# pengsongyou/openscene

Hardware: AMD Instinct MI355X
Metric: active voxels/sec MinkUNet18A fwd+bwd @2cm ScanNet; per-point query ms (higher is better)
Workload: dtype f32 (bf16x6 split-precision MFMA, fp32 accumulate); 1 GPU; ScanNet distillation step (configs[2]): MinkUNet18A, 768-d head, 1 synthetic S100k scene/GPU (100999 voxels on rank 0, 2 cm), training-mode BN; timed = coordinate+kernel maps, forward, cosine loss, backward, gradient all-reduce, Adam step; arch=MinkUNet18A, feature_dim=768, voxels_rank0=100999, parallelism=dp1

## Files before the change

include/openscene_amd.h:

```cpp
#ifndef OPENSCENE_AMD_H
#define OPENSCENE_AMD_H

#include <stddef.h>
#include <stdint.h>

#ifdef __cplusplus
extern "C" {
#endif

#define OSN_OK 0
#define OSN_E_ARG (-1)
#define OSN_E_HIP (-2)
#define OSN_E_WS (-3)
#define OSN_E_RANGE (-4)

typedef void* osn_stream_t;

int osn_version(void);
const char* osn_last_error(void);
int osn_device_ok(void);

int64_t osn_hash_capacity(int64_t n);
size_t osn_coords_unique_ws_bytes(int64_t n);

// ... 460 lines not shown
int osn_net_backward(const osn_net_desc* net, const osn_net_run* run, osn_stream_t stream);
osn_events_t* osn_events_create(int n);
void osn_events_destroy(osn_events_t* e);

#define OSN_MAPS_MAX_STREAMS 4
typedef struct osn_map_level {
    const int32_t* coords4; const uint64_t* keys; const int32_t* vals;
    int64_t cap, rows;
} osn_map_level;
typedef struct osn_map_job {
    int32_t lvl_in, lvl_out;
    int32_t ksize, scale;
    int32_t self_map;
    int32_t stream;
    int32_t bm_fwd, bm_bwd;
    int32_t* nbr_fwd; int32_t* nbr_bwd; int64_t* counts;
    int32_t* order_fwd; int32_t* sorted_fwd; uint32_t* gmask_fwd;
    int32_t* order_bwd; int32_t* sorted_bwd; uint32_t* gmask_bwd;
    void* tl_fwd; void* tl_bwd; void* pl_fwd;
} osn_map_job;
int osn_maps_build(const osn_map_level* levels, int n_levels, const osn_map_job* jobs, int n_jobs,
                   const osn_stream_t* streams, void* const* ws, const uint64_t* ws_bytes, int n_streams,
                   osn_events_t* events);

osn_prof_t* osn_prof_create(int capacity);
void osn_prof_destroy(osn_prof_t* p);
int osn_prof_filter(osn_prof_t* p, const int32_t* tags, int n_tags);
int osn_prof_read(osn_prof_t* p, int32_t* tags, float* ms, int capacity, int reset);

#ifdef __cplusplus
}
#endif
#endif
```

openscene_amd/_lib.py:

```python
import ctypes
import os
import threading

_HERE = os.path.dirname(os.path.abspath(__file__))
LIB_PATH = os.environ.get("OSN_LIB_PATH") or os.path.join(_HERE, "lib", "libopenscene_amd.so")

_c = ctypes
_vp, _i32, _i64, _sz, _f32 = _c.c_void_p, _c.c_int, _c.c_int64, _c.c_size_t, _c.c_float

PROTOTYPES = {
    "osn_version": (_i32, []),
    "osn_last_error": (_c.c_char_p, []),
    "osn_device_ok": (_i32, []),
    "osn_hash_capacity": (_i64, [_i64]),
    "osn_coords_unique_ws_bytes": (_sz, [_i64]),
    "osn_coords_unique": (_i32, [_vp, _i64, _i32, _vp, _vp, _i64, _vp, _vp, _vp, _c.POINTER(_i64), _vp, _sz, _vp]),
    "osn_coords_unique_async": (_i32, [_vp, _i64, _vp, _i32, _vp, _vp, _i64, _vp, _vp, _vp, _vp, _vp, _vp, _sz, _vp]),
    "osn_coords_pyramid_async": (_i32, [_vp, _i64, _vp, _i32, _vp, _vp, _i64, _vp, _vp, _vp, _vp, _vp, _sz, _vp]),
    "osn_kmap_build": (_i32, [_vp, _vp, _i64, _vp, _i64, _i32, _i32, _vp, _vp, _vp]),
    "osn_kmap_build_self": (_i32, [_vp, _vp, _i64, _vp, _i64, _i32, _i32, _vp, _vp, _vp]),
    "osn_kmap_transpose": (_i32, [_vp, _i64, _i32, _i64, _vp, _vp]),
    "osn_kmap_sort_ws_bytes": (_sz, [_i64]),
    "osn_kmap_sort": (_i32, [_vp, _i64, _i32, _vp, _vp, _vp, _vp, _vp, _sz, _vp]),
    "osn_kmap_count": (_i32, [_vp, _i64, _i32, _vp, _vp]),
# ... 47 lines not shown
    "osn_seg_loss_bwd": (_i32, [_vp, _vp, _vp, _i64, _i32, _i64, _vp, _vp, _sz, _vp]),
    "osn_seg_loss_check": (_i32, [_vp, _i64, _i64, _i32, _vp]),
    "osn_seg_vote": (_i32, [_vp, _vp, _i64, _i64, _i32, _vp, _vp]),
    "osn_spconv_fwd_ws_ws_bytes": (_sz, [_i64, _i32, _i32, _i32]),
    "osn_spconv_fwd_ws": (_i32, [_vp, _i64, _vp, _vp, _i64, _i32, _i32, _vp, _vp, _i64, _i32, _i32, _i32, _vp, _sz, _vp]),
    "osn_spconv_wgrad_tl_partial": (_i32, [_vp, _vp, _vp, _i32, _vp, _i64, _i64, _i32, _i32, _i32, _vp, _sz, _vp, _vp]),
    "osn_wgrad_tl_reduce_batch": (_i32, [_vp, _i32, _vp]),
    "osn_stem_conv_fwd": (_i32, [_vp, _vp, _vp, _vp, _i64, _i32, _i32, _i32, _vp]),
    "osn_bn_ws_bytes": (_sz, [_i64, _i32]),
    "osn_bn_stats": (_i32, [_vp, _i64, _i32, _vp, _vp, _vp, _vp, _f32, _vp, _sz, _vp]),
    "osn_bn_apply": (_i32, [_vp, _vp, _vp, _vp, _vp, _f32, _vp, _i32, _vp, _vp, _i64, _i64, _i32, _vp]),
    "osn_spconv_fwd_rg_ok": (_i32, [_i64, _i32, _i32, _i32]),
    "osn_spconv_fwd_rg": (_i32, [_vp, _i64, _vp, _vp, _vp, _vp, _i64, _i32, _i32, _i32, _vp]),
    "osn_bn_forward_train": (_i32, [_vp, _i64, _i32, _vp, _vp, _f32, _vp, _i32, _f32, _vp, _vp, _vp, _vp, _vp, _vp, _i64, _vp, _sz, _vp]),
    "osn_bn_backward": (_i32, [_vp, _vp, _vp, _vp, _i32, _vp, _vp, _vp, _vp, _f32, _i32, _i32, _vp, _vp, _vp, _vp, _i64, _i32,
                               _vp, _sz, _vp]),
    "osn_bn_apply_plan": (_i32, [_i64, _i32, _c.POINTER(_i32), _c.POINTER(_i32)]),
    "osn_bn_set_flat_kernels": (_i32, [_i32]),
    "osn_bn_set_separate_finalize": (_i32, [_i32]),
    "osn_net_plan_query": (_i32, [_vp, _vp, _i32, _vp]),
    "osn_net_forward": (_i32, [_vp, _vp, _vp]),
    "osn_net_backward": (_i32, [_vp, _vp, _vp]),
    "osn_maps_build": (_i32, [_vp, _i32, _vp, _i32, _vp, _vp, _vp, _i32, _vp]),
    "osn_events_create": (_vp, [_i32]),
    "osn_events_destroy": (None, [_vp]),
    "osn_prof_create": (_vp, [_i32]),
    "osn_prof_destroy": (None, [_vp]),
    "osn_prof_filter": (_i32, [_vp, _vp, _i32]),
    "osn_prof_read": (_i32, [_vp, _vp, _vp, _i32, _i32]),
    "osn_relu_fwd": (_i32, [_vp, _vp, _i64, _vp]),
    "osn_relu_bwd": (_i32, [_vp, _vp, _vp, _i64, _vp]),
    "osn_add": (_i32, [_vp, _vp, _vp, _i64, _vp]),
    "osn_cat2": (_i32, [_vp, _i32, _vp, _i32, _vp, _i64, _vp]),
    "osn_cat2_bwd": (_i32, [_vp, _vp, _i32, _vp, _i32, _i64, _vp]),
    "osn_cosine_query": (_i32, [_vp, _vp, _vp, _vp, _vp, _i64, _i32, _i32, _vp]),
    "osn_query_ensemble_ws_bytes": (_sz, [_i64]),
    "osn_query_ensemble": (_i32, [_vp, _vp, _vp, _vp, _vp, _vp, _vp, _vp, _i64, _i32, _i32, _vp, _sz, _vp]),
    "osn_cosine_query_vote": (_i32, [_vp, _vp, _vp, _vp, _vp, _i64, _i32, _i32, _vp]),
    "osn_query_ensemble_vote": (_i32, [_vp, _vp, _vp, _vp, _vp, _vp, _vp, _vp, _i64, _i32, _i32, _vp, _sz, _vp]),
    "osn_eval_confusion": (_i32, [_vp, _vp, _i64, _i32, _vp, _vp, _i64, _vp, _i32, _vp, _vp, _i32, _vp]),
    "osn_eval_check": (_i32, [_vp, _vp]),
    "osn_bank_append": (_i32, [_vp, _i64, _vp, _i64, _i32, _vp, _i64, _vp, _vp]),
    "osn_bank_check": (_i32, [_vp, _vp]),
    "osn_bank_search_ws_bytes": (_sz, [_i64, _i32, _i32, _i32, _i64]),
    "osn_bank_search": (_i32, [_vp, _i64, _i32, _vp, _i32, _i64, _vp, _i32, _i32, _i32, _vp, _vp, _vp, _vp, _vp, _vp, _vp, _sz, _vp]),
    "osn_bank_append_fp8": (_i32, [_vp, _i32, _i64, _vp, _i64, _i32, _vp, _vp, _i64, _vp, _vp]),
# ... 113 lines not shown
```

openscene_amd/csrc/coords.hip:

```cpp
#include "common.h"
#include "coords_impl.h"

namespace osn {

constexpr int SCAN_TPB = 256;
constexpr int SCAN_IPT = 4;
constexpr int SCAN_BLOCK = SCAN_TPB * SCAN_IPT;

__device__ inline int wave_incl_scan(int v, int lane) {
#pragma unroll
    for (int d = 1; d < 64; d <<= 1) {
        int t = __shfl_up(v, d, 64);
        if (lane >= d) v += t;
    }
    return v;
}

template <bool FLAG>
__global__ __launch_bounds__(SCAN_TPB) void scan_block_kernel(const int* __restrict__ in, int* __restrict__ out,
                                                              int* __restrict__ sums, int64_t n,
                                                              const int32_t* __restrict__ n_dev, const int32_t* __restrict__ vals,
                                                              const int32_t* __restrict__ slot_of, int* __restrict__ flag_out) {
    if (n_dev) n = *n_dev;
    __shared__ int wave_tot[SCAN_TPB / 64];
// ... 193 lines not shown
        return;
    }
    int r = -1;
    if (o < n) {
        const int ix = k % ksize, iy = (k / ksize) % ksize, iz = k / (ksize * ksize);
        const int c = ksize / 2;
        const int4 p = coords[o];
        const int x = p.y + (ix - c) * scale, y = p.z + (iy - c) * scale, z = p.w + (iz - c) * scale;
        const int lim = COORD_BIAS - 1;
        if (x >= -lim && x <= lim && y >= -lim && y <= lim && z >= -lim && z <= lim)
            r = table_find(keys, vals, mask, pack_key(p.x, x, y, z));
        nbr[int64_t(k) * n + o] = r;
        if (r >= 0) nbr[int64_t(K - 1 - k) * n + r] = int(o);
    }
    if (counts) {
        const int c = __syncthreads_count(r >= 0);
        if (threadIdx.x == 0 && c) {
            atomicAdd(&counts[k], (unsigned long long)c);
            atomicAdd(&counts[K - 1 - k], (unsigned long long)c);
        }
    }
}

__global__ void kmap_transpose_kernel(const int32_t* __restrict__ nbr, int64_t n_out, int64_t n_in,
                                      int32_t* __restrict__ tbl) {
    const int64_t o = int64_t(blockIdx.x) * blockDim.x + threadIdx.x;
    const int k = blockIdx.y;
    if (o >= n_out) return;
    const int i = nbr[int64_t(k) * n_out + o];
    if (i >= 0) tbl[int64_t(k) * n_in + i] = int(o);
}

__global__ void kmap_count_kernel(const int32_t* __restrict__ nbr, int64_t n_out, unsigned long long* counts) {
    const int k = blockIdx.y;
    int64_t c = 0;
    for (int64_t o = int64_t(blockIdx.x) * blockDim.x + threadIdx.x; o < n_out; o += int64_t(gridDim.x) * blockDim.x)
        c += nbr[int64_t(k) * n_out + o] >= 0;
    __shared__ long long wsum[4];
    for (int d = 32; d >= 1; d >>= 1) c += __shfl_down(c, d, 64);
    if ((threadIdx.x & 63) == 0) wsum[threadIdx.x >> 6] = c;
    __syncthreads();
    if (threadIdx.x == 0) {
        const long long t = wsum[0] + wsum[1] + wsum[2] + wsum[3];
        if (t) atomicAdd(&counts[k], (unsigned long long)t);
    }
}
// ... 219 lines not shown
                                   int64_t* counts, osn_stream_t stream) {
    return kmap_build_self_impl(table_keys, table_vals, cap, coords4, n, ksize, offset_scale, nbr, counts, false, static_cast<hipStream_t>(stream));
}

int osn::kmap_build_self_impl(const uint64_t* table_keys, const int32_t* table_vals, int64_t cap, const int32_t* coords4, int64_t n,
                              int ksize, int offset_scale, int32_t* nbr, int64_t* counts, bool prefilled, hipStream_t st) {
    OSN_REQUIRE(ksize >= 1 && ksize <= 7 && (ksize & 1) == 1, OSN_E_ARG, "osn_kmap_build_self: ksize=%d must be odd, <= 7", ksize);
    OSN_REQUIRE(cap >= 2 && (cap & (cap - 1)) == 0, OSN_E_ARG, "osn_kmap_build_self: cap must be a power of two");
    OSN_REQUIRE(n >= 0, OSN_E_ARG, "osn_kmap_build_self: n < 0");
    const int K = ksize * ksize * ksize;
    if (counts && !prefilled) OSN_HIP(hipMemsetAsync(counts, 0, size_t(K) * 8, st));
    if (n == 0) return OSN_OK;
    OSN_REQUIRE(table_keys && table_vals && coords4 && nbr, OSN_E_ARG, "osn_kmap_build_self: null pointer");
    OSN_REQUIRE(aligned16(coords4), OSN_E_ARG, "osn_kmap_build_self: coords4 must be 16-byte aligned");
    if (K > 1 && !prefilled) OSN_HIP(hipMemsetAsync(nbr + int64_t(K / 2 + 1) * n, 0xFF, size_t(K / 2) * size_t(n) * 4, st));
    const int T = 256;
    hipLaunchKernelGGL(kmap_build_self_kernel, dim3(cdiv(n, T), K / 2 + 1), dim3(T), 0, st, table_keys, table_vals,
                       uint32_t(cap - 1), reinterpret_cast<const int4*>(coords4), n, ksize, offset_scale, nbr,
                       reinterpret_cast<unsigned long long*>(counts));
    OSN_LAUNCH_CHECK();
    return OSN_OK;
}

extern "C" int osn_kmap_transpose(const int32_t* nbr, int64_t n_out, int K, int64_t n_in, int32_t* tbl,
                                  osn_stream_t stream) {
    return kmap_transpose_impl(nbr, n_out, K, n_in, tbl, false, static_cast<hipStream_t>(stream));
}

int osn::kmap_transpose_impl(const int32_t* nbr, int64_t n_out, int K, int64_t n_in, int32_t* tbl, bool prefilled, hipStream_t st) {
    OSN_REQUIRE(K >= 1 && n_out >= 0 && n_in >= 0, OSN_E_ARG, "osn_kmap_transpose: bad sizes");
    if (n_in == 0) return OSN_OK;
    OSN_REQUIRE(tbl, OSN_E_ARG, "osn_kmap_transpose: null tbl");
    if (!prefilled) OSN_HIP(hipMemsetAsync(tbl, 0xFF, size_t(K) * size_t(n_in) * 4, st));
    if (n_out == 0) return OSN_OK;
    OSN_REQUIRE(nbr, OSN_E_ARG, "osn_kmap_transpose: null nbr");
    const int T = 256;
    hipLaunchKernelGGL(kmap_transpose_kernel, dim3(cdiv(n_out, T), K), dim3(T), 0, st, nbr, n_out, n_in, tbl);
    OSN_LAUNCH_CHECK();
    return OSN_OK;
}

extern "C" int osn_kmap_count(const int32_t* nbr, int64_t n_out, int K, int64_t* counts, osn_stream_t stream) {
    hipStream_t st = static_cast<hipStream_t>(stream);
    OSN_REQUIRE(K >= 1 && n_out >= 0 && counts, OSN_E_ARG, "osn_kmap_count: bad arguments");
    OSN_HIP(hipMemsetAsync(counts, 0, size_t(K) * 8, st));
    if (n_out == 0) return OSN_OK;
// ... 10 lines not shown
```

openscene_amd/csrc/coords_impl.h:

```cpp
#pragma once
#include "common.h"

namespace osn {

struct FillJob {
    void* ptr;
    uint64_t bytes;
    uint32_t value;
    uint32_t pad;
};
constexpr int FILL_BATCH = 48;
struct FillJobs {
    FillJob j[FILL_BATCH];
};
int fill_batch(const FillJob* jobs, int n, hipStream_t st);

int kmap_build_impl(const uint64_t* in_table_keys, const int32_t* in_table_vals, int64_t cap, const int32_t* out_coords4, int64_t n_out,
                    int ksize, int offset_scale, int32_t* nbr, int64_t* counts, bool prefilled, hipStream_t st);
int kmap_build_self_impl(const uint64_t* table_keys, const int32_t* table_vals, int64_t cap, const int32_t* coords4, int64_t n, int ksize,
                         int offset_scale, int32_t* nbr, int64_t* counts, bool prefilled, hipStream_t st);
int kmap_transpose_impl(const int32_t* nbr, int64_t n_out, int K, int64_t n_in, int32_t* tbl, bool prefilled, hipStream_t st);

}
```

openscene_amd/csrc/maps.hip:

```cpp
#include "common.h"
#include "events.h"
#include "coords_impl.h"
#include <vector>

using namespace osn;

extern "C" int osn_maps_build(const osn_map_level* levels, int n_levels, const osn_map_job* jobs, int n_jobs,
                              const osn_stream_t* streams, void* const* ws, const uint64_t* ws_bytes, int n_streams,
                              osn_events_t* events) {
    OSN_REQUIRE(levels && jobs && streams && ws && ws_bytes && n_levels >= 1 && n_jobs >= 0 && n_streams >= 1 &&
                    n_streams <= OSN_MAPS_MAX_STREAMS,
                OSN_E_ARG, "osn_maps_build: bad arguments (%d levels, %d jobs, %d streams)", n_levels, n_jobs, n_streams);
    OSN_REQUIRE(n_streams == 1 || (events && events_count(events) >= n_streams + 1), OSN_E_ARG,
                "osn_maps_build: %d streams need an event pool of at least %d events", n_streams, n_streams + 1);
    hipStream_t main = static_cast<hipStream_t>(streams[0]);
    {
        std::vector<FillJob> fills;
        for (int j = 0; j < n_jobs; ++j) {
            const osn_map_job& q = jobs[j];
            if (q.lvl_in < 0 || q.lvl_in >= n_levels || q.lvl_out < 0 || q.lvl_out >= n_levels || q.ksize < 1 || q.ksize > 7 || !q.nbr_fwd) continue;
            const int K = q.ksize * q.ksize * q.ksize;
            const int64_t n_in = levels[q.lvl_in].rows;
            if (q.counts) fills.push_back(FillJob{q.counts, uint64_t(K) * 8u, 0u, 0u});
            if (q.self_map) {
                if (K > 1 && n_in > 0) fills.push_back(FillJob{q.nbr_fwd + int64_t(K / 2 + 1) * n_in, uint64_t(K / 2) * uint64_t(n_in) * 4u, 0xFFFFFFFFu, 0u});
            } else if (q.nbr_bwd && n_in > 0) {
                fills.push_back(FillJob{q.nbr_bwd, uint64_t(K) * uint64_t(n_in) * 4u, 0xFFFFFFFFu, 0u});
            }
        }
        const int rc = fill_batch(fills.data(), int(fills.size()), main);
        if (rc) return rc;
    }
    if (n_streams > 1) {
        hipEvent_t e0 = events_get(events, 0);
        OSN_HIP(hipEventRecord(e0, main));
        for (int s = 1; s < n_streams; ++s) OSN_HIP(hipStreamWaitEvent(static_cast<hipStream_t>(streams[s]), e0, 0));
    }
    bool used[OSN_MAPS_MAX_STREAMS] = {false};
    for (int j = 0; j < n_jobs; ++j) {
        const osn_map_job& q = jobs[j];
        OSN_REQUIRE(q.lvl_in >= 0 && q.lvl_in < n_levels && q.lvl_out >= 0 && q.lvl_out < n_levels && q.ksize >= 1 && q.ksize <= 7,
                    OSN_E_ARG, "osn_maps_build: job %d: levels / kernel size", j);
        const int si = q.stream >= 0 && q.stream < n_streams ? q.stream : 0;
        used[si] = true;
        osn_stream_t st = streams[si];
        const osn_map_level& li = levels[q.lvl_in];
        const osn_map_level& lo = levels[q.lvl_out];
        const int K = q.ksize * q.ksize * q.ksize;
        OSN_REQUIRE(q.nbr_fwd && li.rows >= 1 && lo.rows >= 1, OSN_E_ARG, "osn_maps_build: job %d: null table or empty level", j);
        int rc;
        if (q.self_map) {
            OSN_REQUIRE(q.lvl_in == q.lvl_out && (q.ksize & 1), OSN_E_ARG, "osn_maps_build: job %d: a self map needs one level and an odd kernel", j);
            rc = kmap_build_self_impl(li.keys, li.vals, li.cap, li.coords4, li.rows, q.ksize, q.scale, q.nbr_fwd, q.counts, true,
                                      static_cast<hipStream_t>(st));
        } else {
            rc = kmap_build_impl(li.keys, li.vals, li.cap, lo.coords4, lo.rows, q.ksize, q.scale, q.nbr_fwd, q.counts, true,
                                 static_cast<hipStream_t>(st));
            if (!rc && q.nbr_bwd) rc = kmap_transpose_impl(q.nbr_fwd, lo.rows, K, li.rows, q.nbr_bwd, true, static_cast<hipStream_t>(st));
        }
        if (rc) return rc;
        if (q.sorted_fwd) {
            rc = osn_kmap_sort(q.nbr_fwd, lo.rows, K, q.counts, q.order_fwd, q.sorted_fwd, q.gmask_fwd, ws[si], size_t(ws_bytes[si]), st);
            if (rc) return rc;
        }
        if (q.sorted_bwd) {
            OSN_REQUIRE(q.nbr_bwd, OSN_E_ARG, "osn_maps_build: job %d: tile order of a missing input-gradient table", j);
            rc = osn_kmap_sort(q.nbr_bwd, li.rows, K, q.counts, q.order_bwd, q.sorted_bwd, q.gmask_bwd, ws[si], size_t(ws_bytes[si]), st);
            if (rc) return rc;
        }
        if (q.tl_fwd) {
            rc = osn_tile_lists_build(q.sorted_fwd ? q.sorted_fwd : q.nbr_fwd, lo.rows, K, q.bm_fwd, q.tl_fwd, st);
            if (rc) return rc;
            if (q.pl_fwd) {
                rc = osn_pair_lists_build(q.tl_fwd, q.sorted_fwd ? q.order_fwd : nullptr, lo.rows, K, q.bm_fwd, q.pl_fwd, st);
                if (rc) return rc;
            }
        }
// ... 15 lines not shown
```

openscene_amd/csrc/wgrad_tl.hip:

```cpp
#include "common.h"
#include "split.h"
#include <cstdlib>
#include "pairlist.h"

namespace osn {

typedef short s16x4 __attribute__((ext_vector_type(4)));

__device__ inline int wave_incl_scan_i32(int v, int lane) {
#pragma unroll
    for (int d = 1; d < 64; d <<= 1) {
        const int t = __shfl_up(v, d, 64);
        if (lane >= d) v += t;
    }
    return v;
}

__global__ __launch_bounds__(256) void pair_prefix_kernel(const int32_t* __restrict__ cnt, int n_tiles, int K,
                                                          int32_t* __restrict__ pref, int32_t* __restrict__ total) {
    __shared__ int wtot[4];
    __shared__ int carry_s;
    const int k = blockIdx.x, tid = threadIdx.x, lane = tid & 63, wave = tid >> 6;
    if (tid == 0) carry_s = 0;
    __syncthreads();
    for (int t0 = 0; t0 < n_tiles; t0 += 256) {
        const int t = t0 + tid;
        const int v = t < n_tiles ? cnt[int64_t(t) * K + k] : 0;
        const int incl = wave_incl_scan_i32(v, lane);
        if (lane == 63) wtot[wave] = incl;
        __syncthreads();
        int woff = 0;
#pragma unroll
        for (int w = 0; w < 4; ++w) woff += w < wave ? wtot[w] : 0;
        const int carry = carry_s;
        if (t < n_tiles) pref[int64_t(k) * n_tiles + t] = carry + woff + incl - v;
        __syncthreads();
        if (tid == 255) carry_s = carry + woff + incl;
        __syncthreads();
    }
    if (tid == 0) total[k] = carry_s;
}

__global__ __launch_bounds__(256) void pair_fill_kernel(const int32_t* __restrict__ cnt, const int2* __restrict__ lst,
                                                        const int32_t* __restrict__ out_rows,
                                                        const int32_t* __restrict__ pref, const int32_t* __restrict__ total,
                                                        int n_tiles, int K, int bm, int32_t* __restrict__ pin,
                                                        int32_t* __restrict__ pout, int32_t* __restrict__ poff) {
    __shared__ int poff_s[PL_KMAX + 1];
    const int tid = threadIdx.x, lane = tid & 63, wave = tid >> 6;
    const int64_t tile = blockIdx.x;
    if (wave == 0) {
        int carry = 0;
        for (int k0 = 0; k0 < K; k0 += 64) {
            const int k = k0 + lane;
            const int v = k < K ? total[k] : 0;
            const int incl = wave_incl_scan_i32(v, lane);
            if (k < K) poff_s[k] = carry + incl - v;
            carry += __shfl(incl, 63, 64);
        }
        if (lane == 0) poff_s[K] = carry;
    }
    __syncthreads();
    if (tile == 0)
        for (int k = tid; k <= K; k += 256) poff[k] = poff_s[k];
    for (int k = wave; k < K; k += 4) {
        const int c = cnt[tile * K + k];
        const int base = poff_s[k] + pref[int64_t(k) * n_tiles + tile];
        const int2* src = lst + (tile * K + k) * bm;
        for (int p = lane; p < c; p += 64) {
            const int2 e = src[p];
            pin[base + p] = e.x;
            const int64_t r = tile * bm + e.y;
            pout[base + p] = out_rows ? out_rows[r] : int(r);
        }
    }
}

__global__ __launch_bounds__(256) void pair_plan_kernel(const int32_t* __restrict__ total, int K, int4* __restrict__ items,
                                                        int2* __restrict__ range, int items_max) {
    __shared__ int nk[PL_KMAX];
    __shared__ int start[PL_KMAX + 1];
    __shared__ int quota_s;
    const int tid = threadIdx.x;
    if (tid == 0) {
        long long P = 0;
        for (int k = 0; k < K; ++k) P += total[k];
        long long q = (P + (items_max - K) - 1) / (items_max - K);
        q = (q + 31) / 32 * 32;
        if (q < PL_MIN_QUOTA) q = PL_MIN_QUOTA;
        quota_s = int(q);
    }
    __syncthreads();
    const int quota = quota_s;
    if (tid < K) nk[tid] = (total[tid] + quota - 1) / quota;
    __syncthreads();
    if (tid == 0) {
        int acc = 0;
        for (int k = 0; k < K; ++k) { start[k] = acc; acc += nk[k]; }
        start[K] = acc;
    }
    __syncthreads();
    if (tid < K) range[tid] = make_int2(start[tid], start[tid + 1]);
    for (int t = tid; t < PL_ITEMS; t += 256) {
        int4 it = make_int4(-1, 0, 0, 0);
        if (t < start[K]) {
            int k = 0;
            while (k + 1 < K && start[k + 1] <= t) ++k;
            const int j = t - start[k];
            it.x = k;
            it.y = j * quota;
            it.z = min(it.y + quota, total[k]);
        }
        items[t] = it;
    }
}

template <int MB, int NB, bool BUFG = false>
__global__ __launch_bounds__(256, 2) void wgrad_tl_kernel(const float* __restrict__ rows_a, const float* __restrict__ rows_g,
                                                          const int32_t* __restrict__ idx_a, const int32_t* __restrict__ idx_g,
                                                          const int32_t* __restrict__ poff, const int4* __restrict__ items,
                                                          float* __restrict__ partial, int ca, int cg, int n_cgb,
                                                          int ident_rows, int ident_quota, unsigned a_bytes, unsigned g_bytes) {
    constexpr int CA_T = 32 * MB, CG_T = 32 * NB;
    constexpr int LDA = CA_T + 8, LDG = CG_T + 8;
    constexpr int QA = CA_T / 4, QG = CG_T / 4;
    __shared__ __attribute__((aligned(16))) __bf16 Ap[3][32][LDA];
    __shared__ __attribute__((aligned(16))) __bf16 Gp[3][32][LDG];
    __shared__ int idxbuf[2][32];

    const int tid = threadIdx.x, lane = tid & 63;
    const int wave = __builtin_amdgcn_readfirstlane(tid >> 6);
    const int wi = wave >> 1, wj = wave & 1;
    const int a0 = (blockIdx.x / n_cgb) * CA_T;
    const int g0 = (blockIdx.x % n_cgb) * CG_T;
    int k, p0, p1, base;
    int pstep = 32;
    if (idx_a) {
// ... 218 lines not shown
    return pl_view(nullptr, n_out, K, bm).bytes;
}

extern "C" int osn_pair_lists_build(const void* tl, const int32_t* out_rows, int64_t n_out, int K, int bm, void* pl,
                                    osn_stream_t stream) {
    hipStream_t st = static_cast<hipStream_t>(stream);
    OSN_REQUIRE(n_out >= 0 && n_out < (int64_t(1) << 31), OSN_E_ARG, "osn_pair_lists_build: n_out out of range");
    OSN_REQUIRE(K >= 1 && K <= PL_KMAX && bm >= 1, OSN_E_ARG, "osn_pair_lists_build: K=%d bm=%d", K, bm);
    OSN_REQUIRE(int64_t(K) * n_out < (int64_t(1) << 31), OSN_E_ARG, "osn_pair_lists_build: K * n_out exceeds 32-bit pair indices");
    OSN_REQUIRE(pl, OSN_E_ARG, "osn_pair_lists_build: null pointer");
    PlView v = pl_view(pl, n_out, K, bm);
    if (n_out == 0) {
        OSN_HIP(hipMemsetAsync(pl, 0, PL_OFF_ITEMS, st));
        OSN_HIP(hipMemsetAsync(v.items, 0xFF, size_t(PL_ITEMS) * 16, st));
        OSN_HIP(hipMemsetAsync(v.range, 0, size_t(PL_KMAX) * 8, st));
        return OSN_OK;
    }
    OSN_REQUIRE(tl, OSN_E_ARG, "osn_pair_lists_build: null tile lists");
    const int64_t nt = cdiv(n_out, bm);
    const int32_t* cnt = static_cast<const int32_t*>(tl);
    const int2* lst = reinterpret_cast<const int2*>(static_cast<const char*>(tl) + align_up(size_t(nt) * K * 4, 256));
    hipLaunchKernelGGL(pair_prefix_kernel, dim3(K), dim3(256), 0, st, cnt, int(nt), K, v.pref, v.total);
    const int items_max = PL_ITEMS;
    hipLaunchKernelGGL(pair_plan_kernel, dim3(1), dim3(256), 0, st, v.total, K, v.items, v.range, items_max);
    hipLaunchKernelGGL(pair_fill_kernel, dim3(unsigned(nt)), dim3(256), 0, st, cnt, lst, out_rows, v.pref, v.total, int(nt), K,
                       bm, v.pin, v.pout, v.poff);
    OSN_LAUNCH_CHECK();
    return OSN_OK;
}

namespace {
struct WgTlPlan {
    int mb, nb, n_ab, n_gb;
};
WgTlPlan plan_wg_tl(int ca, int cg) {
    auto blocks = [](int c) { int t = (c + 31) / 32; return t > 4 ? 4 : t; };
    WgTlPlan p;
    p.mb = blocks(ca);
    p.nb = blocks(cg);
    p.n_ab = int(cdiv(ca, 32 * p.mb));
    p.n_gb = int(cdiv(cg, 32 * p.nb));
    return p;
}
int ident_quota(int64_t n) {
    int64_t q = cdiv(n, PL_ITEMS);
    q = (q + 31) / 32 * 32;
    if (q < 64) q = 64;
    return int(q);
}
// ... 142 lines not shown
```

openscene_amd/ops.py:

```python
import ctypes
import os
import threading
import weakref

import torch

from . import _lib
from ._lib import check

_vp = ctypes.c_void_p

_profiler = None


def set_profiler(p):
    global _profiler
    _profiler = p


_raw_stream_of = torch._C._cuda_getCurrentRawStream
_current_device = torch._C._cuda_getDevice


def _prof_start(kind, dev, **meta):
# ... 252 lines not shown

_MAP_LEVEL = None
_MAP_JOB = None
_map_events = {}
MAPS_STREAMS = int(os.environ.get("OSN_MAPS_STREAMS", "1"))


def _map_dtypes():
    global _MAP_LEVEL, _MAP_JOB
    if _MAP_LEVEL is None:
        import numpy as np
        _MAP_LEVEL = np.dtype([("coords4", "<u8"), ("keys", "<u8"), ("vals", "<u8"), ("cap", "<i8"), ("rows", "<i8")])
        _MAP_JOB = np.dtype([(n, "<i4") for n in ("lvl_in", "lvl_out", "ksize", "scale", "self_map", "stream", "bm_fwd", "bm_bwd")] +
                            [(n, "<u8") for n in ("nbr_fwd", "nbr_bwd", "counts", "order_fwd", "sorted_fwd", "gmask_fwd", "order_bwd",
                                                  "sorted_bwd", "gmask_bwd", "tl_fwd", "tl_bwd", "pl_fwd")])
        assert _MAP_LEVEL.itemsize == 40 and _MAP_JOB.itemsize == 128
    return _MAP_LEVEL, _MAP_JOB


def _addr(v):
    return 0 if v is None else (int(v) if isinstance(v, int) else v.data_ptr())


def maps_build(levels, jobs, dev, sort_rows, streams=None):
    import numpy as np
    lib = _prep(dev)
    ldt, jdt = _map_dtypes()
    la = np.zeros(len(levels), dtype=ldt)
    for i, (c, t, rows) in enumerate(levels):
        la[i] = (c.data_ptr(), t.keys.data_ptr(), t.vals.data_ptr(), t.cap, rows)
    ja = np.zeros(max(len(jobs), 1), dtype=jdt)
    for i, q in enumerate(jobs):
        ja[i] = tuple((_addr(q.get(n)) if jdt[n].kind == "u" else int(q.get(n, 0))) for n in jdt.names)
    ns = max(1, min(int(streams) if streams else MAPS_STREAMS, 3))
    idx = _idx(dev)
    main = _stream(dev)
    raws = [main]
    if ns > 1:
        pool = [s for s in (side_stream(dev), aux_stream(dev)) if s.cuda_stream != main]
        ns = min(ns, 1 + len(pool))
        raws += [s.cuda_stream for s in pool[:ns - 1]]
        ev = _map_events.get(idx)
        if ev is None:
            with _Dev(dev):
                ev = _map_events[idx] = lib.osn_events_create(8)
        if not ev:
            ns, raws, ev = 1, [main], None
    else:
        ev = None
    wsb = int(_cached("osn_kmap_sort_ws_bytes", int(sort_rows))) if sort_rows else 256
    wss = [_ws(wsb, dev)] + [ws_on(wsb, dev, r) for r in raws[1:]]
    st_arr = (ctypes.c_void_p * ns)(*raws)
    ws_arr = (ctypes.c_void_p * ns)(*[w.data_ptr() for w in wss])
    wb_arr = (ctypes.c_uint64 * ns)(*[w.numel() for w in wss])
    with _Dev(dev):
        check(lib.osn_maps_build(la.ctypes.data, len(levels), ja.ctypes.data, len(jobs), st_arr, ws_arr, wb_arr, ns, ev),
              "osn_maps_build")


def _w3(weight):
    return weight.unsqueeze(0) if weight.dim() == 2 else weight


def _table_conv(kind, lib, feats, wptr, nbr, n_out, out_rows, gmask, K, cin, cout):
    dev = feats.device
    if nbr is not None:
        if nbr.dtype != torch.int32 or nbr.shape != (K, n_out):
            raise ValueError("nbr must be int32 [%d, %d], got %s %s" % (K, n_out, nbr.dtype, tuple(nbr.shape)))
        nbr = nbr.contiguous()
    elif K != 1 or feats.shape[0] != n_out:
        raise ValueError("nbr=None is the identity map and needs K == 1 and n_in == n_out")
    out = torch.empty((n_out, cout), dtype=torch.float32, device=dev)
    wsb = _cached("osn_spconv_fwd_ws_bytes", n_out, K, cin, cout)
    ws = _ws(wsb, dev) if wsb else None
    tok = _prof_start(kind, dev, n_in=feats.shape[0], n_out=n_out, K=K, cin=cin, cout=cout)
    with _Dev(dev):
        check(getattr(lib, "osn_" + kind)(_p(feats), wptr, _p(nbr), _p(out_rows), _p(gmask), _p(out), n_out, K, cin, cout,
                                          _p(ws), int(wsb), _stream(dev)), "osn_" + kind)
    if tok is not None:
        _profiler.stop(tok)
# ... 2157 lines not shown
```

openscene_amd/sparse.py:

```python
import torch

from . import ops


def _F_mod():
    from . import functional
    return functional


class CoordinateManager:

    PYRAMID = (2, 4, 8, 16)

    def __init__(self, coordinates, pyramid=None):
        pyramid = self.PYRAMID if pyramid is None else tuple(pyramid)
        levels = ops.coords_pyramid(coordinates, (1,) + pyramid)
        coords, inverse, first, table = levels[0]
        self.n_input = coordinates.shape[0]
        self.unique_index = None
        self.inverse_mapping = None
        if coords.shape[0] != coordinates.shape[0]:
            self.unique_index = first.long()
            self.inverse_mapping = inverse.long()
        else:
# ... 107 lines not shown
                continue
            K, n_in, n_out = k ** 3, self.size(si), self.size(so)
            own = si == so
            e = dict(key=key, K=K, n_in=n_in, n_out=n_out, own=own, lane=lane.get((si, so, k), 0), lvl_in=index[si], lvl_out=index[so],
                     ksize=k, scale=si)
            e["nbr_fwd"] = take(4 * K * n_out)
            e["counts"] = take(8 * K)
            if not own:
                e["nbr_bwd"] = take(4 * K * n_in)
            for side, rows, on in (("fwd", n_out, True), ("bwd", n_in, not own)):
                if on and self._want_sort(K, rows):
                    e["order_" + side], e["sorted_" + side] = take(4 * rows), take(4 * K * rows)
                    e["gmask_" + side] = take(4 * ((rows + 31) // 32))
                    sort_rows = max(sort_rows, rows)
                if on and K <= 32:
                    bm = ops.tile_rows(rows)
                    e["bm_" + side] = bm
                    e["tl_" + side] = take(ops._cached("osn_tile_lists_bytes", rows, K, bm))
            if "tl_fwd" in e and (pairs is True or (pairs == "ws" and ((k == 2 and so == 2 * si) or n_out <= _F_mod().WS_MAX_ROWS))):
                e["pl_fwd"] = take(ops._cached("osn_pair_lists_bytes", n_out, K, e["bm_fwd"]))
            plan.append(e)
        if not plan:
            return
        arena = torch.empty(total, dtype=torch.uint8, device=dev)
        base = arena.data_ptr()
        ptr_fields = ("nbr_fwd", "nbr_bwd", "counts", "order_fwd", "sorted_fwd", "gmask_fwd", "order_bwd", "sorted_bwd", "gmask_bwd",
                      "tl_fwd", "tl_bwd", "pl_fwd")
        jobs = []
        for e in plan:
            q = dict(lvl_in=e["lvl_in"], lvl_out=e["lvl_out"], ksize=e["ksize"], scale=e["scale"], self_map=int(e["own"]), stream=e["lane"],
                     bm_fwd=e.get("bm_fwd", 0), bm_bwd=e.get("bm_bwd", 0))
            for f in ptr_fields:
                if f in e:
                    q[f] = base + e[f][0]
            jobs.append(q)
        ops.maps_build([(self._coords[s], self._tables[s], self.size(s)) for s in levels], jobs, dev, sort_rows, streams)

        def view(e, f, dtype, shape):
            off, nb = e[f]
            return arena[off:off + nb].view(dtype).view(shape)
        for e in plan:
            K, n_in, n_out, key = e["K"], e["n_in"], e["n_out"], e["key"]
            nbr = view(e, "nbr_fwd", torch.int32, (K, n_out))
            counts = view(e, "counts", torch.int64, (K,))
            bwd = nbr if e["own"] else view(e, "nbr_bwd", torch.int32, (K, n_in))
            tiles = {}
            for side, rows in (("fwd", n_out), ("bwd", n_in)):
                tiles[side] = (view(e, "order_" + side, torch.int32, (rows,)), view(e, "sorted_" + side, torch.int32, (K, rows)),
                               view(e, "gmask_" + side, torch.int32, ((rows + 31) // 32,))) if ("order_" + side) in e else None
            if e["own"]:
                tiles["bwd"] = tiles["fwd"]
            self._kmaps[key] = (nbr, bwd, bool(e["own"]))
            self._kmaps[("counts",) + key] = counts
            self._kmaps[("tiles",) + key] = (tiles["fwd"], tiles["bwd"])
            if "tl_fwd" in e:
                lf = ops.TileLists(view(e, "tl_fwd", torch.uint8, (e["tl_fwd"][1],)), e["bm_fwd"], n_out, K,
                                   tiles["fwd"][0] if tiles["fwd"] is not None else None)
                lb = lf if e["own"] else ops.TileLists(view(e, "tl_bwd", torch.uint8, (e["tl_bwd"][1],)), e["bm_bwd"], n_in, K,
                                                       tiles["bwd"][0] if tiles["bwd"] is not None else None)
# ... 5 lines not shown
        seen = []

        def walk(v):
            if isinstance(v, torch.Tensor):
                seen.append(v)
            elif isinstance(v, (tuple, list)):
                for u in v:
                    walk(u)
            elif isinstance(v, ops.HashTable):
                walk((v.keys, v.vals))
            elif isinstance(v, ops.TileLists):
                walk((v.buf, v.out_rows))
        for d in (self._coords, self._tables, self._parent, self._kmaps):
            for v in d.values():
                walk(v)
        return seen

    def record_stream(self, stream):
        for t in self.tensors():
            t.record_stream(stream)

    SORT_MIN_ROWS = 8192
    SORT_MIN_ROWS_K8 = 10 ** 9

    def kmap_tiles(self, in_stride, out_stride, ksize, dilation=1):
        key = ("tiles", in_stride, out_stride, ksize, dilation)
        hit = self._kmaps.get(key)
        if hit is not None:
            return hit
        fwd, bwd, flip = self.kmap(in_stride, out_stride, ksize, dilation)
        counts = self.kmap_counts(in_stride, out_stride, ksize, dilation)

        def tiles(tbl):
            if tbl is None or tbl.shape[0] > 32 or tbl.shape[1] < self.SORT_MIN_ROWS:
                return None
            if tbl.shape[0] <= 8 and tbl.shape[1] < self.SORT_MIN_ROWS_K8:
                return None
            return ops.kmap_sort(tbl, counts)

        tf = tiles(fwd)
        tb = tf if (bwd is fwd) else tiles(bwd)
        res = (tf, tb)
        self._kmaps[key] = res
        return res


# ... 155 lines not shown
```

Measured before the change: 12.98 million voxels/s.

## Build self kernel maps via 4x4x4 occupancy bitmap and derive 3x3 from 5x5

Adds an occupancy hash of 64-bit bricks, each bit marking one voxel of a 4x4x4 block. Self kernel-map builds test this bitmap first and probe the main hash table only for offsets that are occupied, which avoids most empty-neighbour lookups. A 3x3x3 self map is copied out of an existing 5x5x5 map on the same level instead of being rebuilt. The pair-plan kernel is also folded into pair_fill, saving one launch. The cost is extra arena memory, a memset of the occupancy table and a fill pass, plus more complex code paths that can be switched off with a legacy flag.

```diff
diff --git a/include/openscene_amd.h b/include/openscene_amd.h
--- a/include/openscene_amd.h
+++ b/include/openscene_amd.h
@@ -506,6 +506,11 @@
 int osn_maps_build(const osn_map_level* levels, int n_levels, const osn_map_job* jobs, int n_jobs,
                    const osn_stream_t* streams, void* const* ws, const uint64_t* ws_bytes, int n_streams,
                    osn_events_t* events);
+size_t osn_maps_occupancy_bytes(int64_t rows);
+int osn_maps_build_occ(const osn_map_level* levels, int n_levels, const osn_map_job* jobs, int n_jobs,
+                       const osn_stream_t* streams, void* const* ws, const uint64_t* ws_bytes, int n_streams,
+                       osn_events_t* events, void* const* occ);
+int osn_maps_set_legacy(int on);
 
 osn_prof_t* osn_prof_create(int capacity);
 void osn_prof_destroy(osn_prof_t* p);
diff --git a/openscene_amd/_lib.py b/openscene_amd/_lib.py
--- a/openscene_amd/_lib.py
+++ b/openscene_amd/_lib.py
@@ -93,6 +93,9 @@
     "osn_net_forward": (_i32, [_vp, _vp, _vp]),
     "osn_net_backward": (_i32, [_vp, _vp, _vp]),
     "osn_maps_build": (_i32, [_vp, _i32, _vp, _i32, _vp, _vp, _vp, _i32, _vp]),
+    "osn_maps_occupancy_bytes": (_sz, [_i64]),
+    "osn_maps_build_occ": (_i32, [_vp, _i32, _vp, _i32, _vp, _vp, _vp, _i32, _vp, _vp]),
+    "osn_maps_set_legacy": (_i32, [_i32]),
     "osn_events_create": (_vp, [_i32]),
     "osn_events_destroy": (None, [_vp]),
     "osn_prof_create": (_vp, [_i32]),
diff --git a/openscene_amd/csrc/coords.hip b/openscene_amd/csrc/coords.hip
--- a/openscene_amd/csrc/coords.hip
+++ b/openscene_amd/csrc/coords.hip
@@ -239,6 +239,128 @@
     }
 }
 
+__global__ void occ_fill_kernel(const int4* __restrict__ coords, int64_t n, int scale, uint64_t* __restrict__ okeys,
+                                unsigned long long* __restrict__ owords, uint32_t omask, int32_t* __restrict__ bad) {
+    const int64_t o = int64_t(blockIdx.x) * blockDim.x + threadIdx.x;
+    if (o >= n) return;
+    const int4 p = coords[o];
+    const int lim = COORD_BIAS - 1;
+    const int xq = floor_div(p.y, scale), yq = floor_div(p.z, scale), zq = floor_div(p.w, scale);
+    if (p.x < 0 || p.x >= 0xFFFF || p.y < -lim || p.y > lim || p.z < -lim || p.z > lim || p.w < -lim || p.w > lim ||
+        xq * scale != p.y || yq * scale != p.z || zq * scale != p.w) {
+        *bad = 1;
+        return;
+    }
+    const uint64_t key = pack_key(p.x, xq >> 2, yq >> 2, zq >> 2);
+    uint32_t slot = hash_key(key) & omask;
+    while (true) {
+        unsigned long long prev = atomicCAS(reinterpret_cast<unsigned long long*>(&okeys[slot]),
+                                            (unsigned long long)KEY_EMPTY, (unsigned long long)key);
+        if (prev == KEY_EMPTY || prev == key) break;
+        slot = (slot + 1) & omask;
+    }
+    atomicOr(&owords[slot], 1ull << ((xq & 3) + 4 * (yq & 3) + 16 * (zq & 3)));
+}
+
+__device__ inline unsigned long long occ_find(const uint64_t* __restrict__ okeys, const unsigned long long* __restrict__ owords,
+                                              uint32_t omask, uint64_t key) {
+    uint32_t slot = hash_key(key) & omask;
+    while (true) {
+        const uint64_t k = okeys[slot];
+        if (k == key) return owords[slot];
+        if (k == KEY_EMPTY) return 0ull;
+        slot = (slot + 1) & omask;
+    }
+}
+
+template <int KS>
+__global__ __launch_bounds__(256) void kmap_build_self_occ_kernel(const uint64_t* __restrict__ keys, const int32_t* __restrict__ vals,
+                                                                  uint32_t mask, const uint64_t* __restrict__ okeys,
+                                                                  const unsigned long long* __restrict__ owords, uint32_t omask,
+                                                                  const int32_t* __restrict__ bad, const int4* __restrict__ coords,
+                                                                  int64_t n, int scale, int32_t* __restrict__ nbr,
+                                                                  unsigned long long* __restrict__ counts) {
+    constexpr int C = KS / 2, K2 = KS * KS, K = K2 * KS;
+    __shared__ int cnt_s[K2];
+    const int tid = threadIdx.x, lane = tid & 63;
+    const int iz = blockIdx.y;
+    const int nk = iz < C ? K2 : K2 / 2;
+    if (tid < K2) cnt_s[tid] = 0;
+    __syncthreads();
+    const int64_t o = int64_t(blockIdx.x) * blockDim.x + tid;
+    const bool live = o < n;
+    int4 p = make_int4(0, 0, 0, 0);
+    uint32_t m = 0;
+    if (live) {
+        p = coords[o];
+        if (*bad) {
+            m = 0xFFFFFFFFu;
+        } else {
+            const int xq = p.y / scale, yq = p.z / scale, zq = p.w / scale;
+            const int zc = zq + iz - C;
+            const int bz = zc >> 2, zb = 16 * (zc & 3);
+            const int bx0 = (xq - C) >> 2, bx1 = (xq + C) >> 2, by0 = (yq - C) >> 2, by1 = (yq + C) >> 2;
+            const unsigned long long w00 = occ_find(okeys, owords, omask, pack_key(p.x, bx0, by0, bz));
+            const unsigned long long w01 = bx1 != bx0 ? occ_find(okeys, owords, omask, pack_key(p.x, bx1, by0, bz)) : w00;
+            const unsigned long long w10 = by1 != by0 ? occ_find(okeys, owords, omask, pack_key(p.x, bx0, by1, bz)) : w00;
+            const unsigned long long w11 = by1 != by0 ? (bx1 != bx0 ? occ_find(okeys, owords, omask, pack_key(p.x, bx1, by1, bz)) : w10) : w01;
+#pragma unroll
+            for (int iy = 0; iy < KS; ++iy) {
+                const int yc = yq + iy - C;
+                const bool jy = (yc >> 2) != by0;
+#pragma unroll
+                for (int ix = 0; ix < KS; ++ix) {
+                    const int xc = xq + ix - C;
+                    const bool jx = (xc >> 2) != bx0;
+                    const unsigned long long w = jy ? (jx ? w11 : w10) : (jx ? w01 : w00);
+                    m |= uint32_t((w >> (zb + 4 * (yc & 3) + (xc & 3))) & 1ull) << (iy * KS + ix);
+                }
+            }
+        }
+    }
+    const int lim = COORD_BIAS - 1;
+    for (int k2 = 0; k2 < nk; ++k2) {
+        int r = -1;
+        if ((m >> k2) & 1u) {
+            const int x = p.y + (k2 % KS - C) * scale, y = p.z + (k2 / KS - C) * scale, z = p.w + (iz - C) * scale;
+            if (x >= -lim && x <= lim && y >= -lim && y <= lim && z >= -lim && z <= lim)
+                r = table_find(keys, vals, mask, pack_key(p.x, x, y, z));
+        }
+        const int k = iz * K2 + k2;
+        if (live) {
+            nbr[int64_t(k) * n + o] = r;
+            if (r >= 0) nbr[int64_t(K - 1 - k) * n + r] = int(o);
+        }
+        const unsigned long long b = __ballot(r >= 0);
+        if (lane == 0 && b) atomicAdd(&cnt_s[k2], __popcll(b));
+    }
+    if (iz == C) {
+        if (live) nbr[int64_t(K / 2) * n + o] = int(o);
+        if (counts && blockIdx.x == 0 && tid == 0) counts[K / 2] = (unsigned long long)n;
+    }
+    __syncthreads();
+    if (counts && tid < nk) {
+        const int c = cnt_s[tid];
+        if (c) {
+            const int k = iz * K2 + tid;
+            atomicAdd(&counts[k], (unsigned long long)c);
+            atomicAdd(&counts[K - 1 - k], (unsigned long long)c);
+        }
+    }
+}
+
+__global__ void kmap_derive_self_kernel(const int32_t* __restrict__ nbr_big, const unsigned long long* __restrict__ counts_big,
+                                        int kbig, int64_t n, int ksize, int32_t* __restrict__ nbr,
+                                        unsigned long long* __restrict__ counts) {
+    const int64_t o = int64_t(blockIdx.x) * blockDim.x + threadIdx.x;
+    const int k = blockIdx.y;
+    const int d = (kbig - ksize) / 2;
+    const int ix = k % ksize, iy = (k / ksize) % ksize, iz = k / (ksize * ksize);
+    const int kb = (ix + d) + kbig * ((iy + d) + kbig * (iz + d));
+    if (o < n) nbr[int64_t(k) * n + o] = nbr_big[int64_t(kb) * n + o];
+    if (counts && blockIdx.x == 0 && threadIdx.x == 0) counts[k] = counts_big[kb];
+}
+
 __global__ void kmap_transpose_kernel(const int32_t* __restrict__ nbr, int64_t n_out, int64_t n_in,
                                       int32_t* __restrict__ tbl) {
     const int64_t o = int64_t(blockIdx.x) * blockDim.x + threadIdx.x;
@@ -504,6 +626,50 @@
     return OSN_OK;
 }
 
+int osn::occ_fill_impl(const OccView& occ, const int32_t* coords4, int64_t n, int scale, hipStream_t st) {
+    OSN_REQUIRE(n >= 1 && n < (int64_t(1) << 31) && scale >= 1 && coords4 && aligned16(coords4) && occ.bad && occ.cap >= 2 * n &&
+                    (reinterpret_cast<uintptr_t>(occ.bad) & 7u) == 0,
+                OSN_E_ARG, "occ_fill: bad arguments (%lld rows, scale %d)", (long long)n, scale);
+    const int T = 256;
+    hipLaunchKernelGGL(occ_fill_kernel, dim3(cdiv(n, T)), dim3(T), 0, st, reinterpret_cast<const int4*>(coords4), n, scale, occ.keys,
+                       occ.words, uint32_t(occ.cap - 1), occ.bad);
+    OSN_LAUNCH_CHECK();
+    return OSN_OK;
+}
+
+int osn::kmap_build_self_occ_impl(const uint64_t* table_keys, const int32_t* table_vals, int64_t cap, const OccView& occ,
+                                  const int32_t* coords4, int64_t n, int ksize, int offset_scale, int32_t* nbr, int64_t* counts,
+                                  hipStream_t st) {
+    OSN_REQUIRE(ksize == 3 || ksize == 5, OSN_E_ARG, "kmap_build_self_occ: ksize=%d", ksize);
+    OSN_REQUIRE(cap >= 2 && (cap & (cap - 1)) == 0 && n >= 1 && offset_scale >= 1, OSN_E_ARG, "kmap_build_self_occ: cap / rows / scale");
+    OSN_REQUIRE(table_keys && table_vals && coords4 && nbr && occ.bad && aligned16(coords4), OSN_E_ARG, "kmap_build_self_occ: null pointer");
+    const int T = 256;
+    const dim3 grid(cdiv(n, T), ksize / 2 + 1);
+    const int4* c4 = reinterpret_cast<const int4*>(coords4);
+    unsigned long long* cnt = reinterpret_cast<unsigned long long*>(counts);
+    if (ksize == 3)
+        hipLaunchKernelGGL(kmap_build_self_occ_kernel<3>, grid, dim3(T), 0, st, table_keys, table_vals, uint32_t(cap - 1), occ.keys,
+                           occ.words, uint32_t(occ.cap - 1), occ.bad, c4, n, offset_scale, nbr, cnt);
+    else
+        hipLaunchKernelGGL(kmap_build_self_occ_kernel<5>, grid, dim3(T), 0, st, table_keys, table_vals, uint32_t(cap - 1), occ.keys,
+                           occ.words, uint32_t(occ.cap - 1), occ.bad, c4, n, offset_scale, nbr, cnt);
+    OSN_LAUNCH_CHECK();
+    return OSN_OK;
+}
+
+int osn::kmap_derive_self_impl(const int32_t* nbr_big, const int64_t* counts_big, int ksize_big, int64_t n, int ksize, int32_t* nbr,
+                               int64_t* counts, hipStream_t st) {
+    OSN_REQUIRE(ksize >= 1 && (ksize & 1) && (ksize_big & 1) && ksize < ksize_big && ksize_big <= 7, OSN_E_ARG,
+                "kmap_derive_self: kernel %d out of kernel %d", ksize, ksize_big);
+    OSN_REQUIRE(n >= 1 && nbr_big && nbr && (counts_big || !counts), OSN_E_ARG, "kmap_derive_self: null pointer or no rows");
+    const int T = 256;
+    hipLaunchKernelGGL(kmap_derive_self_kernel, dim3(cdiv(n, T), ksize * ksize * ksize), dim3(T), 0, st, nbr_big,
+                       reinterpret_cast<const unsigned long long*>(counts_big), ksize_big, n, ksize, nbr,
+                       reinterpret_cast<unsigned long long*>(counts));
+    OSN_LAUNCH_CHECK();
+    return OSN_OK;
+}
+
 extern "C" int osn_kmap_transpose(const int32_t* nbr, int64_t n_out, int K, int64_t n_in, int32_t* tbl,
                                   osn_stream_t stream) {
     return kmap_transpose_impl(nbr, n_out, K, n_in, tbl, false, static_cast<hipStream_t>(stream));
diff --git a/openscene_amd/csrc/coords_impl.h b/openscene_amd/csrc/coords_impl.h
--- a/openscene_amd/csrc/coords_impl.h
+++ b/openscene_amd/csrc/coords_impl.h
@@ -19,6 +19,35 @@
                     int ksize, int offset_scale, int32_t* nbr, int64_t* counts, bool prefilled, hipStream_t st);
 int kmap_build_self_impl(const uint64_t* table_keys, const int32_t* table_vals, int64_t cap, const int32_t* coords4, int64_t n, int ksize,
                          int offset_scale, int32_t* nbr, int64_t* counts, bool prefilled, hipStream_t st);
+int kmap_derive_self_impl(const int32_t* nbr_big, const int64_t* counts_big, int ksize_big, int64_t n, int ksize, int32_t* nbr,
+                          int64_t* counts, hipStream_t st);
+struct OccView {
+    int32_t* bad;
+    unsigned long long* words;
+    uint64_t* keys;
+    int64_t cap;
+    size_t bytes;
+};
+inline int64_t occ_capacity(int64_t rows) {
+    int64_t cap = 1024;
+    while (cap < 2 * rows) cap <<= 1;
+    return cap;
+}
+inline OccView occ_view(void* base, int64_t rows) {
+    OccView v;
+    char* p = static_cast<char*>(base);
+    v.cap = occ_capacity(rows);
+    v.bad = reinterpret_cast<int32_t*>(p);
+    v.words = reinterpret_cast<unsigned long long*>(p + 256);
+    v.keys = reinterpret_cast<uint64_t*>(p + 256 + size_t(v.cap) * 8);
+    v.bytes = 256 + size_t(v.cap) * 16;
+    return v;
+}
+int occ_fill_impl(const OccView& occ, const int32_t* coords4, int64_t n, int scale, hipStream_t st);
+int kmap_build_self_occ_impl(const uint64_t* table_keys, const int32_t* table_vals, int64_t cap, const OccView& occ,
+                             const int32_t* coords4, int64_t n, int ksize, int offset_scale, int32_t* nbr, int64_t* counts,
+                             hipStream_t st);
+bool maps_legacy();
 int kmap_transpose_impl(const int32_t* nbr, int64_t n_out, int K, int64_t n_in, int32_t* tbl, bool prefilled, hipStream_t st);
 
 }
diff --git a/openscene_amd/csrc/maps.hip b/openscene_amd/csrc/maps.hip
--- a/openscene_amd/csrc/maps.hip
+++ b/openscene_amd/csrc/maps.hip
@@ -1,23 +1,67 @@
 #include "common.h"
 #include "events.h"
 #include "coords_impl.h"
+#include <atomic>
 #include <vector>
 
 using namespace osn;
 
+static std::atomic<int> g_maps_legacy{0};
+bool osn::maps_legacy() { return g_maps_legacy.load(std::memory_order_relaxed) != 0; }
+extern "C" int osn_maps_set_legacy(int on) { return g_maps_legacy.exchange(on ? 1 : 0); }
+
+extern "C" size_t osn_maps_occupancy_bytes(int64_t rows) { return occ_view(nullptr, rows > 0 ? rows : 1).bytes; }
+
 extern "C" int osn_maps_build(const osn_map_level* levels, int n_levels, const osn_map_job* jobs, int n_jobs,
                               const osn_stream_t* streams, void* const* ws, const uint64_t* ws_bytes, int n_streams,
                               osn_events_t* events) {
+    return osn_maps_build_occ(levels, n_levels, jobs, n_jobs, streams, ws, ws_bytes, n_streams, events, nullptr);
+}
+
+extern "C" int osn_maps_build_occ(const osn_map_level* levels, int n_levels, const osn_map_job* jobs, int n_jobs,
+                                  const osn_stream_t* streams, void* const* ws, const uint64_t* ws_bytes, int n_streams,
+                                  osn_events_t* events, void* const* occ) {
     OSN_REQUIRE(levels && jobs && streams && ws && ws_bytes && n_levels >= 1 && n_jobs >= 0 && n_streams >= 1 &&
                     n_streams <= OSN_MAPS_MAX_STREAMS,
                 OSN_E_ARG, "osn_maps_build: bad arguments (%d levels, %d jobs, %d streams)", n_levels, n_jobs, n_streams);
     OSN_REQUIRE(n_streams == 1 || (events && events_count(events) >= n_streams + 1), OSN_E_ARG,
                 "osn_maps_build: %d streams need an event pool of at least %d events", n_streams, n_streams + 1);
     hipStream_t main = static_cast<hipStream_t>(streams[0]);
+    std::vector<int> from(size_t(n_jobs > 0 ? n_jobs : 0), -1);
+    if (!maps_legacy())
+        for (int j = 0; j < n_jobs; ++j) {
+            const osn_map_job& q = jobs[j];
+            if (!q.self_map || q.ksize != 3 || !q.nbr_fwd) continue;
+            for (int i = 0; i < j && from[j] < 0; ++i) {
+                const osn_map_job& b = jobs[i];
+                if (b.self_map && b.ksize == 5 && b.lvl_in == q.lvl_in && b.lvl_out == q.lvl_out && b.scale == q.scale && b.nbr_fwd &&
+                    (b.counts || !q.counts) && b.lvl_in >= 0 && b.lvl_in < n_levels && b.lvl_in == b.lvl_out)
+                    from[j] = i;
+            }
+        }
+    std::vector<int> occ_job(size_t(n_levels), -1);
+    auto lane_of = [&](const osn_map_job& q) { return q.stream >= 0 && q.stream < n_streams ? q.stream : 0; };
+    auto occ_source = [&](int j) -> int {
+        const osn_map_job& q = jobs[j];
+        if (!occ || maps_legacy() || from[j] >= 0 || !q.self_map || (q.ksize != 3 && q.ksize != 5) || !q.nbr_fwd || q.scale < 1 ||
+            q.lvl_in < 0 || q.lvl_in >= n_levels || q.lvl_in != q.lvl_out || !occ[q.lvl_in] || levels[q.lvl_in].rows < 1)
+            return -1;
+        const int s = occ_job[size_t(q.lvl_in)];
+        if (s < 0) return j;
+        return jobs[s].scale == q.scale && lane_of(jobs[s]) == lane_of(q) ? s : -1;
+    };
     {
         std::vector<FillJob> fills;
         for (int j = 0; j < n_jobs; ++j) {
+            if (occ_source(j) != j) continue;
+            occ_job[size_t(jobs[j].lvl_in)] = j;
+            const OccView v = occ_view(occ[jobs[j].lvl_in], levels[jobs[j].lvl_in].rows);
+            fills.push_back(FillJob{v.bad, 256u + uint64_t(v.cap) * 8u, 0u, 0u});
+            fills.push_back(FillJob{v.keys, uint64_t(v.cap) * 8u, 0xFFFFFFFFu, 0u});
+        }
+        for (int j = 0; j < n_jobs; ++j) {
             const osn_map_job& q = jobs[j];
+            if (from[j] >= 0) continue;
             if (q.lvl_in < 0 || q.lvl_in >= n_levels || q.lvl_out < 0 || q.lvl_out >= n_levels || q.ksize < 1 || q.ksize > 7 || !q.nbr_fwd) continue;
             const int K = q.ksize * q.ksize * q.ksize;
             const int64_t n_in = levels[q.lvl_in].rows;
@@ -41,7 +85,8 @@
         const osn_map_job& q = jobs[j];
         OSN_REQUIRE(q.lvl_in >= 0 && q.lvl_in < n_levels && q.lvl_out >= 0 && q.lvl_out < n_levels && q.ksize >= 1 && q.ksize <= 7,
                     OSN_E_ARG, "osn_maps_build: job %d: levels / kernel size", j);
-        const int si = q.stream >= 0 && q.stream < n_streams ? q.stream : 0;
+        const osn_map_job& qs = from[j] >= 0 ? jobs[from[j]] : q;
+        const int si = qs.stream >= 0 && qs.stream < n_streams ? qs.stream : 0;
         used[si] = true;
         osn_stream_t st = streams[si];
         const osn_map_level& li = levels[q.lvl_in];
@@ -51,8 +96,17 @@
         int rc;
         if (q.self_map) {
             OSN_REQUIRE(q.lvl_in == q.lvl_out && (q.ksize & 1), OSN_E_ARG, "osn_maps_build: job %d: a self map needs one level and an odd kernel", j);
-            rc = kmap_build_self_impl(li.keys, li.vals, li.cap, li.coords4, li.rows, q.ksize, q.scale, q.nbr_fwd, q.counts, true,
-                                      static_cast<hipStream_t>(st));
+            if (from[j] >= 0)
+                rc = kmap_derive_self_impl(qs.nbr_fwd, qs.counts, qs.ksize, li.rows, q.ksize, q.nbr_fwd, q.counts, static_cast<hipStream_t>(st));
+            else if (const int os = occ_source(j); os >= 0) {
+                const OccView v = occ_view(occ[q.lvl_in], li.rows);
+                rc = os == j ? occ_fill_impl(v, li.coords4, li.rows, q.scale, static_cast<hipStream_t>(st)) : OSN_OK;
+                if (!rc)
+                    rc = kmap_build_self_occ_impl(li.keys, li.vals, li.cap, v, li.coords4, li.rows, q.ksize, q.scale, q.nbr_fwd, q.counts,
+                                                  static_cast<hipStream_t>(st));
+            } else
+                rc = kmap_build_self_impl(li.keys, li.vals, li.cap, li.coords4, li.rows, q.ksize, q.scale, q.nbr_fwd, q.counts, true,
+                                          static_cast<hipStream_t>(st));
         } else {
             rc = kmap_build_impl(li.keys, li.vals, li.cap, lo.coords4, lo.rows, q.ksize, q.scale, q.nbr_fwd, q.counts, true,
                                  static_cast<hipStream_t>(st));
diff --git a/openscene_amd/csrc/wgrad_tl.hip b/openscene_amd/csrc/wgrad_tl.hip
--- a/openscene_amd/csrc/wgrad_tl.hip
+++ b/openscene_amd/csrc/wgrad_tl.hip
@@ -2,6 +2,7 @@
 #include "split.h"
 #include <cstdlib>
 #include "pairlist.h"
+#include "coords_impl.h"
 
 namespace osn {
 
@@ -41,11 +42,15 @@
     if (tid == 0) total[k] = carry_s;
 }
 
+__device__ inline void pair_plan(const int32_t* __restrict__ total, int K, int4* __restrict__ items, int2* __restrict__ range,
+                                 int items_max);
+
 __global__ __launch_bounds__(256) void pair_fill_kernel(const int32_t* __restrict__ cnt, const int2* __restrict__ lst,
                                                         const int32_t* __restrict__ out_rows,
                                                         const int32_t* __restrict__ pref, const int32_t* __restrict__ total,
                                                         int n_tiles, int K, int bm, int32_t* __restrict__ pin,
-                                                        int32_t* __restrict__ pout, int32_t* __restrict__ poff) {
+                                                        int32_t* __restrict__ pout, int32_t* __restrict__ poff, int4* __restrict__ items,
+                                                        int2* __restrict__ range, int items_max) {
     __shared__ int poff_s[PL_KMAX + 1];
     const int tid = threadIdx.x, lane = tid & 63, wave = tid >> 6;
     const int64_t tile = blockIdx.x;
@@ -74,10 +79,11 @@
             pout[base + p] = out_rows ? out_rows[r] : int(r);
         }
     }
-}
-
-__global__ __launch_bounds__(256) void pair_plan_kernel(const int32_t* __restrict__ total, int K, int4* __restrict__ items,
-                                                        int2* __restrict__ range, int items_max) {
+    if (tile == 0 && items) pair_plan(total, K, items, range, items_max);
+}
+
+__device__ inline void pair_plan(const int32_t* __restrict__ total, int K, int4* __restrict__ items, int2* __restrict__ range,
+                                 int items_max) {
     __shared__ int nk[PL_KMAX];
     __shared__ int start[PL_KMAX + 1];
     __shared__ int quota_s;
@@ -113,6 +119,11 @@
         }
         items[t] = it;
     }
+}
+
+__global__ __launch_bounds__(256) void pair_plan_kernel(const int32_t* __restrict__ total, int K, int4* __restrict__ items,
+                                                        int2* __restrict__ range, int items_max) {
+    pair_plan(total, K, items, range, items_max);
 }
 
 template <int MB, int NB, bool BUFG = false>
@@ -377,9 +388,10 @@
     const int2* lst = reinterpret_cast<const int2*>(static_cast<const char*>(tl) + align_up(size_t(nt) * K * 4, 256));
     hipLaunchKernelGGL(pair_prefix_kernel, dim3(K), dim3(256), 0, st, cnt, int(nt), K, v.pref, v.total);
     const int items_max = PL_ITEMS;
-    hipLaunchKernelGGL(pair_plan_kernel, dim3(1), dim3(256), 0, st, v.total, K, v.items, v.range, items_max);
+    const bool own_plan = maps_legacy();
+    if (own_plan) hipLaunchKernelGGL(pair_plan_kernel, dim3(1), dim3(256), 0, st, v.total, K, v.items, v.range, items_max);
     hipLaunchKernelGGL(pair_fill_kernel, dim3(unsigned(nt)), dim3(256), 0, st, cnt, lst, out_rows, v.pref, v.total, int(nt), K,
-                       bm, v.pin, v.pout, v.poff);
+                       bm, v.pin, v.pout, v.poff, own_plan ? nullptr : v.items, v.range, items_max);
     OSN_LAUNCH_CHECK();
     return OSN_OK;
 }
diff --git a/openscene_amd/ops.py b/openscene_amd/ops.py
--- a/openscene_amd/ops.py
+++ b/openscene_amd/ops.py
@@ -298,7 +298,7 @@
     return 0 if v is None else (int(v) if isinstance(v, int) else v.data_ptr())
 
 
-def maps_build(levels, jobs, dev, sort_rows, streams=None):
+def maps_build(levels, jobs, dev, sort_rows, streams=None, occ=None):
     import numpy as np
     lib = _prep(dev)
     ldt, jdt = _map_dtypes()
@@ -329,9 +329,18 @@
     st_arr = (ctypes.c_void_p * ns)(*raws)
     ws_arr = (ctypes.c_void_p * ns)(*[w.data_ptr() for w in wss])
     wb_arr = (ctypes.c_uint64 * ns)(*[w.numel() for w in wss])
-    with _Dev(dev):
-        check(lib.osn_maps_build(la.ctypes.data, len(levels), ja.ctypes.data, len(jobs), st_arr, ws_arr, wb_arr, ns, ev),
+    occ_arr = (ctypes.c_void_p * len(levels))(*[_addr(o) or None for o in occ]) if occ is not None else None
+    with _Dev(dev):
+        check(lib.osn_maps_build_occ(la.ctypes.data, len(levels), ja.ctypes.data, len(jobs), st_arr, ws_arr, wb_arr, ns, ev, occ_arr),
               "osn_maps_build")
+
+
+def maps_occupancy_bytes(rows):
+    return int(_cached("osn_maps_occupancy_bytes", int(rows)))
+
+
+def maps_set_legacy(on):
+    return bool(_lib.load().osn_maps_set_legacy(int(bool(on))))
 
 
 def _w3(weight):
diff --git a/openscene_amd/sparse.py b/openscene_amd/sparse.py
--- a/openscene_amd/sparse.py
+++ b/openscene_amd/sparse.py
@@ -153,6 +153,10 @@
             plan.append(e)
         if not plan:
             return
+        occ = {}
+        for e in plan:
+            if e["own"] and e["ksize"] in (3, 5) and e["lvl_in"] not in occ:
+                occ[e["lvl_in"]] = take(ops.maps_occupancy_bytes(e["n_in"])) if e["n_in"] * (e["K"] // 2) >= self.OCC_MIN_PROBES else None
         arena = torch.empty(total, dtype=torch.uint8, device=dev)
         base = arena.data_ptr()
         ptr_fields = ("nbr_fwd", "nbr_bwd", "counts", "order_fwd", "sorted_fwd", "gmask_fwd", "order_bwd", "sorted_bwd", "gmask_bwd",
@@ -165,7 +169,8 @@
                 if f in e:
                     q[f] = base + e[f][0]
             jobs.append(q)
-        ops.maps_build([(self._coords[s], self._tables[s], self.size(s)) for s in levels], jobs, dev, sort_rows, streams)
+        ops.maps_build([(self._coords[s], self._tables[s], self.size(s)) for s in levels], jobs, dev, sort_rows, streams,
+                       occ=[base + occ[i][0] if occ.get(i) else None for i in range(len(levels))])
 
         def view(e, f, dtype, shape):
             off, nb = e[f]
@@ -217,6 +222,7 @@
 
     SORT_MIN_ROWS = 8192
     SORT_MIN_ROWS_K8 = 10 ** 9
+    OCC_MIN_PROBES = 400000
 
     def kmap_tiles(self, in_stride, out_stride, ksize, dilation=1):
         key = ("tiles", in_stride, out_stride, ksize, dilation)
```

New measurement: 13.26 million voxels/s (median of 6 runs). +2.1%, better.
